# MMAThijssen/catfish

Hardware: AMD Instinct MI355X
Metric: signal samples/s classified (higher is better)
Workload: dtype f32

## Files before the change

catfish_amd/build.py:

```python
from __future__ import annotations

import json
import os
import re
import shutil
import subprocess
import sys

_HERE = os.path.dirname(os.path.abspath(__file__))
SRC = os.path.join(_HERE, "csrc", "catfish_hip.hip")
OUT = os.path.join(_HERE, "csrc", "libcatfish_hip.so")
HEADER = os.path.join(os.path.dirname(_HERE), "include", "catfish_hip.h")


def hipcc_path():
    for cand in (os.environ.get("HIPCC"), shutil.which("hipcc"), "/opt/rocm/bin/hipcc"):
        if cand and os.path.exists(cand):
            return cand
    raise RuntimeError("hipcc not found (set HIPCC or install ROCm)")


def needs_build():
    if not os.path.exists(OUT):
        return True
    csrc = os.path.dirname(SRC)
    deps = [HEADER] + [os.path.join(csrc, f) for f in os.listdir(csrc) if f.endswith((".hip", ".hpp", ".h"))]
    newest = max(os.path.getmtime(p) for p in deps)
    return os.path.getmtime(OUT) < newest


RESOURCES = os.path.join(_HERE, "csrc", "kernel_resources.json")
_REMARK = re.compile(r"remark:\s+(Function Name|TotalSGPRs|VGPRs|AGPRs|ScratchSize \[bytes/lane\]|Occupancy \[waves/SIMD\]|SGPRs Spill|"
                     r"VGPRs Spill|LDS Size \[bytes/block\]):\s*(\S+)")
_KEYS = {"TotalSGPRs": "sgprs", "VGPRs": "vgprs", "AGPRs": "agprs", "ScratchSize [bytes/lane]": "scratch_bytes_per_lane",
         "Occupancy [waves/SIMD]": "waves_per_simd", "SGPRs Spill": "sgpr_spills", "VGPRs Spill": "vgpr_spills",
         "LDS Size [bytes/block]": "lds_bytes"}


def parse_resource_remarks(text):
    out, cur = {}, None
    for m in _REMARK.finditer(text):
        key, val = m.group(1), m.group(2)
        if key == "Function Name":
            cur = out.setdefault(val, {})
        elif cur is not None:
            try:
                cur[_KEYS[key]] = int(val)
            except ValueError:
                pass
    return out


def demangle(names):
    tool = next((t for t in ("/opt/rocm/lib/llvm/bin/llvm-cxxfilt", shutil.which("c++filt")) if t and os.path.exists(t)), None)
    names = list(names)
    if tool is None or not names:
        return dict(zip(names, names))
    res = subprocess.run([tool], input="\n".join(names) + "\n", stdout=subprocess.PIPE, universal_newlines=True)
    got = res.stdout.splitlines()
    return dict(zip(names, got)) if res.returncode == 0 and len(got) == len(names) else dict(zip(names, names))


def check_resources(resources):
    bad = []
    for name, r in sorted(resources.items()):
        if r.get("scratch_bytes_per_lane", 0) != 0 or r.get("vgpr_spills", 0) != 0:
            bad.append("%s: scratch %s B/lane, %s VGPR spills" % (name, r.get("scratch_bytes_per_lane"), r.get("vgpr_spills")))
        if r.get("vgprs", 0) + r.get("agprs", 0) > 512:
            bad.append("%s: %s VGPRs + %s AGPRs exceed the 512-register file" % (name, r.get("vgprs"), r.get("agprs")))
    return bad


def build_native(force=False, verbose=False):
    if not force and not needs_build():
        return OUT
    cmd = [hipcc_path(), "--offload-arch=gfx950", "-O3", "-std=c++17", "-fPIC", "-shared", "-mllvm", "-amdgpu-mfma-vgpr-form",
           "-Rpass-analysis=kernel-resource-usage", "-o", OUT + ".tmp", SRC]
    if verbose:
        print(" ".join(cmd))
    res = subprocess.run(cmd, stdout=subprocess.PIPE, stderr=subprocess.STDOUT, universal_newlines=True)
    if res.returncode != 0:
        if os.path.exists(OUT + ".tmp"):
            os.unlink(OUT + ".tmp")
        raise RuntimeError("hipcc failed:\n" + "\n".join(l for l in res.stdout.splitlines() if "kernel-resource-usage" not in l))
    resources = parse_resource_remarks(res.stdout)
    names = demangle(resources)
    record = {"flags": cmd[1:-3], "kernels": {names[k]: v for k, v in sorted(resources.items())}}
    bad = check_resources(record["kernels"])
    if bad or not resources:
        os.unlink(OUT + ".tmp")
        raise RuntimeError("hipcc built kernels that spill (or reported no kernel resources at all):\n  " + "\n  ".join(bad))
    with open(RESOURCES, "w") as fh:
        json.dump(record, fh, indent=1, sort_keys=True)
        fh.write("\n")
    os.replace(OUT + ".tmp", OUT)
    return OUT


if __name__ == "__main__":
    print(build_native(force="--force" in sys.argv, verbose=True))
```

catfish_amd/csrc/catfish_hip.hip:

```cpp
#include <hip/hip_runtime.h>
#include <stdint.h>
#include <string.h>
#include <stdio.h>
#include <vector>
#include <string>
#include <cmath>
#include <mutex>
#include <set>
#include <functional>

#include "../../include/catfish_hip.h"

typedef float f32x4 __attribute__((ext_vector_type(4)));
typedef float f32x2 __attribute__((ext_vector_type(2)));

#define CF_T 35
#define CF_H 64
#define CF_C 32
#define CF_TILE 16

#define MFMA16(a, b, c) __builtin_amdgcn_mfma_f32_16x16x4f32((a), (b), (c), 0, 0, 0)

#ifndef CF_ABLATE
#define CF_ABLATE 0
#endif
#ifndef CF_PREFETCH
#define CF_PREFETCH 1
#endif

__device__ __forceinline__ float cf_sigmoid(float x) {
    return __builtin_amdgcn_rcpf(1.0f + __expf(-x));
}
__device__ __forceinline__ float cf_tanh(float x) {
    return fmaf(-2.0f, __builtin_amdgcn_rcpf(1.0f + __expf(2.0f * x)), 1.0f);
}
#define CF_GATE_SCALE (-1.4426950408889634)
#define CF_CAND_SCALE (2.8853900817779268)
__device__ __forceinline__ float cf_sigmoid_pre(float a) {
    return __builtin_amdgcn_rcpf(1.0f + __builtin_amdgcn_exp2f(a));
}
__device__ __forceinline__ float cf_tanh_pre(float a) {
    return fmaf(-2.0f, __builtin_amdgcn_rcpf(1.0f + __builtin_amdgcn_exp2f(a)), 1.0f);
}
__device__ __forceinline__ f32x2 cf_sigmoid_pre2(f32x2 a) {
    f32x2 e = {__builtin_amdgcn_exp2f(a.x), __builtin_amdgcn_exp2f(a.y)};
    e = e + (f32x2){1.0f, 1.0f};
    return (f32x2){__builtin_amdgcn_rcpf(e.x), __builtin_amdgcn_rcpf(e.y)};
}
__device__ __forceinline__ f32x2 cf_tanh_pre2(f32x2 a) {
    return __builtin_elementwise_fma((f32x2){-2.0f, -2.0f}, cf_sigmoid_pre2(a), (f32x2){1.0f, 1.0f});
}
template <typename T>
struct far_lds {
    static constexpr int N64K = 65536 / sizeof(T);
    const T *b0, *b1, *b2;
    __device__ __forceinline__ explicit far_lds(const T* base) {
        int o1 = N64K, o2 = 2 * N64K;
        asm volatile("" : "+v"(o1), "+v"(o2));
        b0 = base; b1 = base + o1; b2 = base + o2;
    }
    __device__ __forceinline__ const T& operator[](int e) const { return e < N64K ? b0[e] : (e < 2 * N64K ? b1[e - N64K] : b2[e - 2 * N64K]); }
};
__device__ __forceinline__ f32x4 cf_sigmoid_pre4(f32x4 a) {
    f32x4 e = {__builtin_amdgcn_exp2f(a.x), __builtin_amdgcn_exp2f(a.y), __builtin_amdgcn_exp2f(a.z), __builtin_amdgcn_exp2f(a.w)};
    e = e + (f32x4){1.0f, 1.0f, 1.0f, 1.0f};
    return (f32x4){__builtin_amdgcn_rcpf(e.x), __builtin_amdgcn_rcpf(e.y), __builtin_amdgcn_rcpf(e.z), __builtin_amdgcn_rcpf(e.w)};
}
__device__ __forceinline__ f32x4 cf_tanh_pre4(f32x4 a) {
    return __builtin_elementwise_fma((f32x4){-2.0f, -2.0f, -2.0f, -2.0f}, cf_sigmoid_pre4(a), (f32x4){1.0f, 1.0f, 1.0f, 1.0f});
}
struct cf_dropout {
    float keep_prob = 1.f;
    uint32_t seed = 0;
    int32_t layer = 0;
    const double* step = nullptr;
};
__device__ __forceinline__ uint32_t cf_fmix32(uint32_t v) {
    v ^= v >> 16; v *= 0x85ebca6bu; v ^= v >> 13; v *= 0xc2b2ae35u; v ^= v >> 16;
    return v;
}
__device__ __forceinline__ uint32_t cf_drop_key(const cf_dropout& d) {
    const uint32_t st = d.step ? (uint32_t)(long long)d.step[0] : 0u;
    return cf_fmix32(d.seed ^ cf_fmix32(0x9E3779B9u * (uint32_t)(d.layer + 1) + st * 0x85ebca6bu));
}
__device__ __forceinline__ f32x4 cf_drop_scale4(uint32_t key, float keep_prob, int64_t idx4) {
    const uint32_t thresh = (uint32_t)fminf(keep_prob * 4294967296.0f, 4294967040.0f);
    const float inv = 1.0f / keep_prob;
    const uint64_t e = (uint64_t)idx4 * 4u;
    const uint32_t base = (uint32_t)e ^ ((uint32_t)(e >> 32) * 0x9E3779B9u);
    f32x4 o;
    o.x = cf_fmix32((base + 0u) ^ key) < thresh ? inv : 0.f;
    o.y = cf_fmix32((base + 1u) ^ key) < thresh ? inv : 0.f;
    o.z = cf_fmix32((base + 2u) ^ key) < thresh ? inv : 0.f;
    o.w = cf_fmix32((base + 3u) ^ key) < thresh ? inv : 0.f;
    return o;
}

__device__ __forceinline__ f32x4 relu4(f32x4 v) {
    f32x4 o;
    o.x = fmaxf(v.x, 0.f); o.y = fmaxf(v.y, 0.f); o.z = fmaxf(v.z, 0.f); o.w = fmaxf(v.w, 0.f);
    return o;
}

__host__ __device__ constexpr int gru_x_floats(int cin) { return (cin / 4) * 3 * 256; }
__host__ __device__ constexpr int gru_hg_floats() { return 16 * 2 * 256; }
__host__ __device__ constexpr int gru_hc_floats() { return 16 * 256; }
__host__ __device__ constexpr int gru_bias_off(int cin) { return gru_x_floats(cin) + gru_hg_floats() + gru_hc_floats(); }
__host__ __device__ constexpr int gru_dense_off(int cin) { return gru_bias_off(cin) + 192; }
__host__ __device__ constexpr int gru_pack_floats(int cin) { return gru_dense_off(cin) + 64; }
#define CF_GRU_MAX_WAVES 8
// ... 135 lines not shown
    if (!CHUNKED) t_chunks = 1;
    const int chunk_len = CHUNKED ? (CF_T + t_chunks - 1) / t_chunks : CF_T;
    for (int task = blockIdx.x * waves_per_block + wave; task < n_tiles * t_chunks; task += gridDim.x * waves_per_block) {
        const int tile = CHUNKED ? task / t_chunks : task;
        const int p0 = CHUNKED ? (task - tile * t_chunks) * chunk_len : 0;
        const int p1 = CHUNKED ? min(p0 + chunk_len, CF_T) : CF_T;
        if (CHUNKED && p0 >= p1) continue;
        {
            const int64_t base = (int64_t)tile * CF_TILE * CF_T;
            const int64_t limit = n_windows * CF_T;
            for (int i = lane; i < CF_TILE * CF_T; i += 64) xs[i] = (base + i < limit) ? x_nat[base + i] : 0.f;
            __builtin_amdgcn_fence(__ATOMIC_RELEASE, "wavefront");
            __builtin_amdgcn_wave_barrier();
            __builtin_amdgcn_fence(__ATOMIC_ACQUIRE, "wavefront");
        }
        f32x4 w_sc[2], b_sc[2], w_f[2], b_f[2];
#pragma unroll
        for (int mo = 0; mo < 2; ++mo) { w_sc[mo] = vec0(2, mo); b_sc[mo] = vec0(3, mo); w_f[mo] = vec0(4, mo); b_f[mo] = vec0(5, mo); }
        f32x4 a_pp[2] = {zero, zero}, a_p[2] = {zero, zero}, a_sp[2] = {zero, zero};
        f32x4 b_pp[2] = {zero, zero}, b_p[2] = {zero, zero}, b_sp[2] = {zero, zero};
        for (int i = p0 > 2 ? p0 - 2 : 0; i <= p1 + 1; ++i) {
            f32x4 a_c[2] = {zero, zero}, a_sc[2] = {zero, zero};
            if (i < CF_T) {
                const float xv = xs[(lane & 15) * CF_T + i];
#pragma unroll
                for (int mo = 0; mo < 2; ++mo) {
                    a_sc[mo] = w_sc[mo] * xv + b_sc[mo];
                    a_c[mo] = relu4(w_f[mo] * xv + b_f[mo]);
                }
            }
            f32x4 y0[2] = {zero, zero};
            const bool have_y0 = i >= 1 && i <= CF_T && i >= p0;
            if (have_y0) {
                f32x4 acc[2] = {vec0(0, 0), vec0(0, 1)};
                unit_mma(w0 + 0 * 1024, lane, a_pp, acc);
                unit_mma(w0 + 1 * 1024, lane, a_p, acc);
                unit_mma(w0 + 2 * 1024, lane, a_c, acc);
                f32x4 o2[2] = {relu4(acc[0]), relu4(acc[1])};
                f32x4 acc3[2] = {vec0(1, 0), vec0(1, 1)};
                unit_mma(w0 + 3 * 1024, lane, o2, acc3);
                y0[0] = relu4(relu4(acc3[0]) + a_sp[0]);
                y0[1] = relu4(relu4(acc3[1]) + a_sp[1]);
                if (CHUNKED && y0_frag && i - 1 >= p0 && i - 1 < p1) {
                    f32x4* d0 = y0_frag + ((int64_t)tile * CF_T + (i - 1)) * 2 * 64 + lane;
                    d0[0] = y0[0];
                    d0[64] = y0[1];
                }
            }
            f32x4 b_c[2] = {zero, zero}, b_sc[2] = {zero, zero};
            if (have_y0) {
                b_sc[0] = vec1(0, 0); b_sc[1] = vec1(0, 1);
                unit_mma(w1 + 0 * 1024, lane, y0, b_sc);
                f32x4 acc[2] = {vec1(1, 0), vec1(1, 1)};
                unit_mma(w1 + 1 * 1024, lane, y0, acc);
                b_c[0] = relu4(acc[0]); b_c[1] = relu4(acc[1]);
            }
            if (i >= 2 && i - 2 >= p0 && i - 2 < p1) {
                f32x4 acc[2] = {vec1(2, 0), vec1(2, 1)};
                unit_mma(w1 + 2 * 1024, lane, b_pp, acc);
                unit_mma(w1 + 3 * 1024, lane, b_p, acc);
                unit_mma(w1 + 4 * 1024, lane, b_c, acc);
                f32x4 o2[2] = {relu4(acc[0]), relu4(acc[1])};
                f32x4 acc3[2] = {vec1(3, 0), vec1(3, 1)};
                unit_mma(w1 + 5 * 1024, lane, o2, acc3);
                f32x4* dst = y_frag + ((int64_t)tile * CF_T + (i - 2)) * 2 * 64 + lane;
                dst[0] = relu4(relu4(acc3[0]) + b_sp[0]);
                dst[64] = relu4(relu4(acc3[1]) + b_sp[1]);
            }
#pragma unroll
            for (int mo = 0; mo < 2; ++mo) {
                a_pp[mo] = a_p[mo]; a_p[mo] = a_c[mo]; a_sp[mo] = a_sc[mo];
                if (i >= 1) { b_pp[mo] = b_p[mo]; b_p[mo] = b_c[mo]; b_sp[mo] = b_sc[mo]; }
            }
        }
        __builtin_amdgcn_wave_barrier();
    }
}

template <int CIN>
__device__ __forceinline__ void gru_stage_weights(float* lds, const float* __restrict__ wpack, int dir) {
    constexpr int PACK = gru_pack_floats(CIN);
    const f32x4* src = reinterpret_cast<const f32x4*>(wpack + (size_t)dir * PACK);
    f32x4* dst = reinterpret_cast<f32x4*>(lds);
    for (int i = threadIdx.x; i < PACK / 4; i += blockDim.x) dst[i] = src[i];
}

#ifndef CF_SCHED_DS_FIRST
#define CF_SCHED_DS_FIRST 1
#endif
#if CF_SCHED_DS_FIRST
#define CF_KSTEP_SCHED(nds, nmfma)                               \
    __builtin_amdgcn_sched_group_barrier(0x100, nds, 0);         \
    __builtin_amdgcn_sched_group_barrier(0x008, nmfma, 0);       \
    __builtin_amdgcn_sched_barrier(0)
#else
#define CF_KSTEP_SCHED(nds, nmfma) __builtin_amdgcn_sched_barrier(0)
#endif
template <int CIN, bool LAST, bool STASH = false>
__device__ __forceinline__ void gru_tile(const float* lds, int lane, int dir, int tile, const f32x4* __restrict__ X,
                                         f32x4* __restrict__ Y, float* __restrict__ P, int n_tiles,
                                         f32x4* __restrict__ S = nullptr, f32x4* __restrict__ YD = nullptr, cf_dropout drop = cf_dropout(),
                                         int s_begin = 0, int s_end = CF_T, f32x4* HO = nullptr) {
    const uint32_t drop_key = (STASH && YD) ? cf_drop_key(drop) : 0u;
    constexpr int KGX = CIN / 16;
    constexpr int KSX = CIN / 4;
    constexpr int XN4 = gru_x_floats(CIN) / 4;
    constexpr int HG4 = gru_hg_floats() / 4;
    constexpr int BIAS = gru_bias_off(CIN);
    constexpr int DENSE = gru_dense_off(CIN);
    const int q = lane >> 4;
    const f32x4* WX = reinterpret_cast<const f32x4*>(lds) + lane;
    const far_lds<f32x4> WL(WX);
    const f32x4* B4 = reinterpret_cast<const f32x4*>(lds + BIAS) + q;
    const f32x4* D4 = reinterpret_cast<const f32x4*>(lds + DENSE) + q;
    {
        f32x4 h[4] = {{0, 0, 0, 0}, {0, 0, 0, 0}, {0, 0, 0, 0}, {0, 0, 0, 0}};
        if (s_begin > 0) {
#pragma unroll
            for (int m = 0; m < 4; ++m) h[m] = HO[m * 64 + lane];
        }
        f32x4 xc[KGX];
        {
            const int t0 = dir ? (CF_T - 1 - s_begin) : s_begin;
            const f32x4* src = X + ((int64_t)tile * CF_T + t0) * KGX * 64 + lane;
#pragma unroll
            for (int g = 0; g < KGX; ++g) xc[g] = src[g * 64];
        }
        for (int s = s_begin; s < s_end; ++s) {
            const int t = dir ? (CF_T - 1 - s) : s;
            f32x4 acc[12];
#pragma unroll
            for (int mo = 0; mo < 12; ++mo) acc[mo] = B4[mo * 4];
            constexpr int PF = CF_PREFETCH;
            auto loadA = [&](int p, f32x4 (&d)[3]) {
                if (p < KSX) { d[0] = WL[(p * 3 + 0) * 64]; d[1] = WL[(p * 3 + 1) * 64]; d[2] = WL[(p * 3 + 2) * 64]; }
                else if (p < KSX + 16) { d[0] = WL[XN4 + ((p - KSX) * 2 + 0) * 64]; d[1] = WL[XN4 + ((p - KSX) * 2 + 1) * 64]; }
                else if (p < KSX + 32) { d[0] = WL[XN4 + HG4 + (p - KSX - 16) * 64]; }
            };
            f32x4 ac[3], an[3], a2[3];
            loadA(0, ac);
            if (PF == 2) loadA(1, an);
#pragma unroll
            for (int ks = 0; ks < KSX; ++ks) {
                if (PF == 2) loadA(ks + 2, a2); else loadA(ks + 1, an);
                const float b = xc[ks >> 2][ks & 3];
#pragma unroll
                for (int g = 0; g < 3; ++g) {
                    acc[4 * g + 0] = MFMA16(ac[g].x, b, acc[4 * g + 0]);
                    acc[4 * g + 1] = MFMA16(ac[g].y, b, acc[4 * g + 1]);
                    acc[4 * g + 2] = MFMA16(ac[g].z, b, acc[4 * g + 2]);
                    acc[4 * g + 3] = MFMA16(ac[g].w, b, acc[4 * g + 3]);
                }
                CF_KSTEP_SCHED(3, 12);
#pragma unroll
                for (int g = 0; g < 3; ++g) { ac[g] = an[g]; if (PF == 2) an[g] = a2[g]; }
            }
            {
                int tn = dir ? (t - 1) : (t + 1);
                tn = tn < 0 ? 0 : (tn > CF_T - 1 ? CF_T - 1 : tn);
                const f32x4* src = X + ((int64_t)tile * CF_T + tn) * KGX * 64 + lane;
#pragma unroll
                for (int g = 0; g < KGX; ++g) if (!(CF_ABLATE & 2)) xc[g] = src[g * 64];
            }
#pragma unroll
            for (int ks = 0; ks < 16; ++ks) {
                if (PF == 2) loadA(KSX + ks + 2, a2); else loadA(KSX + ks + 1, an);
                const float b = h[ks >> 2][ks & 3];
#pragma unroll
                for (int g = 0; g < 2; ++g) {
                    acc[4 * g + 0] = MFMA16(ac[g].x, b, acc[4 * g + 0]);
                    acc[4 * g + 1] = MFMA16(ac[g].y, b, acc[4 * g + 1]);
                    acc[4 * g + 2] = MFMA16(ac[g].z, b, acc[4 * g + 2]);
                    acc[4 * g + 3] = MFMA16(ac[g].w, b, acc[4 * g + 3]);
                }
                CF_KSTEP_SCHED(2, 8);
                ac[0] = an[0]; ac[1] = an[1];
                if (PF == 2) { an[0] = a2[0]; an[1] = a2[1]; }
            }
            f32x4 rh[4];
#pragma unroll
            for (int m = 0; m < 4; ++m) {
                if (CF_ABLATE & 1) { rh[m] = acc[m] * 0.001f; continue; }
                const f32x4 rv = cf_sigmoid_pre4(acc[m]);
                rh[m] = rv * h[m];
                if constexpr (STASH) acc[m] = rv;
            }
#pragma unroll
            for (int ks = 0; ks < 16; ++ks) {
                if (PF == 2) loadA(KSX + 16 + ks + 2, a2); else loadA(KSX + 16 + ks + 1, an);
                const float b = rh[ks >> 2][ks & 3];
                acc[8] = MFMA16(ac[0].x, b, acc[8]);
                acc[9] = MFMA16(ac[0].y, b, acc[9]);
                acc[10] = MFMA16(ac[0].z, b, acc[10]);
                acc[11] = MFMA16(ac[0].w, b, acc[11]);
                CF_KSTEP_SCHED(1, 4);
                ac[0] = an[0];
                if (PF == 2) an[0] = a2[0];
            }
#pragma unroll
            for (int m = 0; m < 4; ++m) {
                if (CF_ABLATE & 1) { h[m] = acc[4 + m] * 0.001f + acc[8 + m] * 0.001f; continue; }
                const f32x4 u = cf_sigmoid_pre4(acc[4 + m]);
                const f32x4 c = cf_tanh_pre4(acc[8 + m]);
                h[m] = __builtin_elementwise_fma(u, h[m] - c, c);
                if constexpr (STASH) { acc[4 + m] = u; acc[8 + m] = c; }
            }
            if constexpr (STASH) {
                f32x4* sdst = S + (((int64_t)tile * CF_T + t) * 2 + dir) * 12 * 64 + lane;
#pragma unroll
                for (int j = 0; j < 12; ++j) sdst[j * 64] = acc[j];
            }
            if constexpr (!LAST) {
                f32x4* dst = Y + (((int64_t)tile * CF_T + t) * 8 + dir * 4) * 64 + lane;
#pragma unroll
                for (int m = 0; m < 4; ++m) if (!(CF_ABLATE & 2) || s == CF_T - 1) dst[m * 64] = h[m];
                if constexpr (STASH) {
                    if (YD) {
                        const int64_t i0 = (((int64_t)tile * CF_T + t) * 8 + dir * 4) * 64 + lane;
#pragma unroll
                        for (int m = 0; m < 4; ++m) YD[i0 + m * 64] = h[m] * cf_drop_scale4(drop_key, drop.keep_prob, i0 + m * 64);
                    }
                }
            } else {
                float pm[4];
#pragma unroll
                for (int m = 0; m < 4; ++m) {
                    const f32x4 wd = D4[m * 4];
                    pm[m] = wd.x * h[m].x;
                    pm[m] = fmaf(wd.y, h[m].y, pm[m]); pm[m] = fmaf(wd.z, h[m].z, pm[m]); pm[m] = fmaf(wd.w, h[m].w, pm[m]);
                }
                float p = ((pm[0] + pm[1]) + pm[2]) + pm[3];
                p += __shfl_xor(p, 16);
                p += __shfl_xor(p, 32);
                if (lane < 16) P[(((int64_t)dir * n_tiles + tile) * CF_T + t) * 16 + lane] = p;
            }
            __builtin_amdgcn_sched_barrier(0);
        }
        if (s_end < CF_T) {
#pragma unroll
            for (int m = 0; m < 4; ++m) HO[m * 64 + lane] = h[m];
        }
    }
}

__device__ __forceinline__ void cf_handoff_publish(unsigned* flag) {
    asm volatile("s_waitcnt vmcnt(0)" ::: "memory");
    __builtin_amdgcn_fence(__ATOMIC_RELEASE, "workgroup");
    asm volatile("s_waitcnt vmcnt(0)" ::: "memory");
    __hip_atomic_store(flag, 1u, __ATOMIC_RELAXED, __HIP_MEMORY_SCOPE_WORKGROUP);
}
__device__ __forceinline__ void cf_handoff_wait(unsigned* flag, int lane, unsigned* err) {
    if (lane == 0) {
        bool ok = false;
        for (int it = 0; it < 1000000 && !ok; ++it) {
            ok = __hip_atomic_load(flag, __ATOMIC_RELAXED, __HIP_MEMORY_SCOPE_WORKGROUP) != 0u;
            if (!ok) __builtin_amdgcn_s_sleep(16);
        }
        if (!ok && err) __hip_atomic_store(err, 1u, __ATOMIC_RELAXED, __HIP_MEMORY_SCOPE_SYSTEM);
    }
    __builtin_amdgcn_fence(__ATOMIC_ACQUIRE, "workgroup");
    asm volatile("s_waitcnt vmcnt(0)" ::: "memory");
}

template <int CIN, bool LAST>
__global__ __launch_bounds__(512, 2) void gru_layer_kernel(const float* __restrict__ wpack,
                                                           const f32x4* __restrict__ X,
                                                           f32x4* __restrict__ Y,
                                                           float* __restrict__ P,
                                                           int n_tiles,
                                                           int balance,
                                                           f32x4* hand,
                                                           unsigned* err) {
    extern __shared__ __attribute__((aligned(16))) float lds[];
    const int dir = blockIdx.y;
    gru_stage_weights<CIN>(lds, wpack, dir);
    unsigned* flags = reinterpret_cast<unsigned*>(lds + gru_pack_floats(CIN));
    if (threadIdx.x < CF_GRU_MAX_WAVES) flags[threadIdx.x] = 0u;
    __syncthreads();
    const int lane = threadIdx.x & 63;
    const int wave = __builtin_amdgcn_readfirstlane(threadIdx.x >> 6);
    const int nwaves = blockDim.x >> 6;
    const int t0 = (int)((int64_t)blockIdx.x * n_tiles / gridDim.x);
    const int t1 = (int)((int64_t)(blockIdx.x + 1) * n_tiles / gridDim.x);
    cf_gru_share sh;
    int n_pieces;
    if (balance) {
        sh = cf_gru_balanced_share(t1 - t0, nwaves, wave, CF_T);
        n_pieces = (sh.head_end > 0) + sh.whole_count + (sh.tail_begin < CF_T);
    } else {
        sh.head_tile = sh.head_end = 0; sh.whole_first = sh.whole_count = 0; sh.tail_tile = 0; sh.tail_begin = CF_T;
        n_pieces = t1 - t0 > wave ? (t1 - t0 - wave + nwaves - 1) / nwaves : 0;
    }
    f32x4* slots = hand + ((size_t)(dir * gridDim.x + blockIdx.x) * CF_GRU_MAX_WAVES) * 4 * 64;
    const int has_head = balance && sh.head_end > 0;
    for (int i = 0; i < n_pieces; ++i) {
        int tile, s_begin = 0, s_end = CF_T;
        f32x4* ho = nullptr;
        if (!balance) {
            tile = t0 + wave + i * nwaves;
        } else if (i < has_head) {
            tile = t0 + sh.head_tile; s_end = sh.head_end; ho = slots + wave * 4 * 64;
        } else if (i < has_head + sh.whole_count) {
            tile = t0 + sh.whole_first + (i - has_head);
        } else {
            tile = t0 + sh.tail_tile; s_begin = sh.tail_begin; ho = slots + (wave - 1) * 4 * 64;
            cf_handoff_wait(flags + (wave - 1), lane, err);
        }
        gru_tile<CIN, LAST>(lds, lane, dir, tile, X, Y, P, n_tiles, nullptr, nullptr, cf_dropout(), s_begin, s_end, ho);
        if (s_end < CF_T) cf_handoff_publish(flags + wave);
    }
}

struct cf_fused_args {
    const float* w[3];
    const f32x4* x0;
    f32x4* y[2];
    float* p;
    unsigned* flags;
    int lds_floats;
    unsigned* err;
    int n_tiles;
    int groups;
    int n_layers;
    int cin0;
// ... 792 lines not shown
    *idx = m->ev_pending.size() - 1;
    return CF_OK;
}
static int prof_end(cf_model* m, hipStream_t s, size_t idx) {
    if (!m->prof) return CF_OK;
    HIP_TRY(hipEventRecord(m->ev_pending[idx].b, s));
    return CF_OK;
}

static int pick_waves(int n_tile_tasks, int n_cu) {
    int w = (n_tile_tasks + n_cu - 1) / n_cu;
    return w <= 1 ? 1 : (w <= 2 ? 2 : (w <= 4 ? 4 : 8));
}

static bool use_coop(const cf_model* m, int n_tiles) {
    static const int coop_env = cf_knob("CATFISH_COOP") ? atoi(cf_knob("CATFISH_COOP")) : -1;
    const bool coop = coop_env >= 0 ? coop_env != 0 : n_tiles <= m->n_cu;
    return coop && !(CF_ABLATE & 4) && n_tiles <= m->n_cu;
}

template <int CIN>
static void launch_xproj(cf_model* m, const float* wpack, const float* X, int n_tiles, hipStream_t s) {
    const int lds_env = cf_knob("CATFISH_XPROJ_LDS") ? atoi(cf_knob("CATFISH_XPROJ_LDS")) : 1;
    if (lds_env) {
        int chunks = cf_xproj_plan(n_tiles, m->n_cu, CIN);
        if (cf_knob("CATFISH_XPROJ_CHUNKS")) {
            const int c = std::max(1, std::min(CF_T, atoi(cf_knob("CATFISH_XPROJ_CHUNKS"))));
            const int tl = (CF_T + c - 1) / c;
            chunks = (CF_T + tl - 1) / tl;
        }
        hipLaunchKernelGGL((gru_xproj_lds_kernel<CIN>), dim3(n_tiles * chunks, 2), dim3(256), gru_x_floats(CIN) * 4, s, wpack,
                           reinterpret_cast<const f32x4*>(X), reinterpret_cast<f32x4*>(m->d_xp), n_tiles, chunks);
    } else {
        hipLaunchKernelGGL((gru_xproj_kernel<CIN>), dim3(n_tiles * cf_xproj_chunks(n_tiles), 2), dim3(256), 0, s, wpack,
                           reinterpret_cast<const f32x4*>(X), reinterpret_cast<f32x4*>(m->d_xp), n_tiles, cf_xproj_chunks(n_tiles));
    }
}

template <int CIN, bool LAST>
static int launch_gru(cf_model* m, const float* wpack, const float* X, float* Y, float* P, int n_tiles, hipStream_t s, int slot,
                      float* hand = nullptr) {
    if (use_coop(m, n_tiles)) {
        size_t pi = 0;
        int rc = prof_begin(m, slot, s, &pi);
        if (rc != CF_OK) return rc;
        const int gx = std::min(n_tiles, std::max(1, m->n_cu / 2));
        const f32x4* xp = nullptr;
        if (CIN >= 32 && n_tiles <= m->xp_tiles) {
            xp = reinterpret_cast<const f32x4*>(m->d_xp);
            launch_xproj<CIN>(m, wpack, X, n_tiles, s);
        }
        hipLaunchKernelGGL((gru_layer_coop_kernel<CIN, LAST>), dim3(gx, 2), dim3(256), (gru_pack_floats(CIN) + CF_COOP_XCH_FLOATS) * 4, s,
                           wpack, reinterpret_cast<const f32x4*>(X), reinterpret_cast<f32x4*>(Y), P, n_tiles, xp);
        HIP_TRY(hipGetLastError());
        return prof_end(m, s, pi);
    }
    static const int waves_env = cf_knob("CATFISH_WAVES") ? atoi(cf_knob("CATFISH_WAVES")) : 0;
    const int waves = waves_env > 0 ? std::min(waves_env, 8) : ((CF_ABLATE & 4) ? 4 : pick_waves(2 * n_tiles, m->n_cu));
    const int groups = (n_tiles + waves - 1) / waves;
    int per_dir = m->n_cu / 2 > 0 ? m->n_cu / 2 : 1;
    constexpr int lds_bytes = gru_pack_floats(CIN) * 4;
    if (lds_bytes <= 80 * 1024) per_dir *= 2;
    int gx = groups < per_dir ? groups : per_dir;
    size_t pi = 0;
    int rc = prof_begin(m, slot, s, &pi);
    if (rc != CF_OK) return rc;
    int balance = 0;
    if (hand) {
        const int wg_per_cu = std::max(1, (2 * gx + m->n_cu - 1) / m->n_cu);
        const int gx_one = std::max(1, m->n_cu / 2);
        const int load_rr = cf_gru_grid_load(n_tiles, gx, waves, wg_per_cu, CF_T, 0);
        const int load_bal = cf_gru_grid_load(n_tiles, gx, waves, wg_per_cu, CF_T, 1);
        const int load_one = gx > gx_one ? cf_gru_grid_load(n_tiles, gx_one, waves, 1, CF_T, 1) : -1;
        const char* env = cf_knob("CATFISH_GRU_BALANCE");
        const int forced = env ? atoi(env) : -1;
        int best = load_rr;
        if (forced < 0 ? (load_bal >= 0 && load_bal < best) : (forced >= 1 && load_bal >= 0)) { balance = 1; best = load_bal; }
        if (forced < 0 ? (load_one >= 0 && load_one < best) : (forced == 2 && load_one >= 0)) { balance = 1; gx = gx_one; }
    }
    hipLaunchKernelGGL((gru_layer_kernel<CIN, LAST>), dim3(gx, 2), dim3(waves * 64), lds_bytes + CF_GRU_MAX_WAVES * 4, s, wpack,
                       reinterpret_cast<const f32x4*>(X), reinterpret_cast<f32x4*>(Y), P, n_tiles, balance, reinterpret_cast<f32x4*>(hand),
                       m->d_err);
    HIP_TRY(hipGetLastError());
    return prof_end(m, s, pi);
}

template <int CIN, bool LAST, int NP>
static int launch_gru_bf16(cf_model* m, const char* wpack, const float* X, float* Y, float* P, int n_tiles32, hipStream_t s, int slot) {
    static const int waves_env = cf_knob("CATFISH_BF16_WAVES") ? atoi(cf_knob("CATFISH_BF16_WAVES")) : 0;
    static const int wgs_env = cf_knob("CATFISH_BF16_WGS") ? atoi(cf_knob("CATFISH_BF16_WGS")) : 0;
    const int waves = waves_env > 0 ? std::min(waves_env, 8) : pick_waves(2 * n_tiles32, m->n_cu);
    const int groups = (n_tiles32 + waves - 1) / waves;
    int per_dir = m->n_cu / 2 > 0 ? m->n_cu / 2 : 1;
    constexpr int lds_bytes = gb_pack_bytes(CIN, NP);
    if (lds_bytes <= 80 * 1024) per_dir *= 2;
    if (wgs_env > 0) per_dir = wgs_env;
    const int gx = groups < per_dir ? groups : per_dir;
    size_t pi = 0;
    int rc = prof_begin(m, slot, s, &pi);
    if (rc != CF_OK) return rc;
    const int pipe_env = cf_knob("CATFISH_BF16_PIPE") ? atoi(cf_knob("CATFISH_BF16_PIPE")) : 1;
    if constexpr (NP == 1) {
        if (pipe_env) {
            hipLaunchKernelGGL((gru_bf16_pipe_kernel<CIN, LAST>), dim3(gx, 2), dim3(waves * 64), lds_bytes, s, wpack,
                               reinterpret_cast<const bf16x8*>(X), reinterpret_cast<bf16x8*>(Y), P, n_tiles32);
            HIP_TRY(hipGetLastError());
            return prof_end(m, s, pi);
        }
    }
    if constexpr (NP == 2) {
        if (pipe_env) {
            const int w4 = std::min(waves, 4);
            const int g4 = (n_tiles32 + w4 - 1) / w4;
            const int per4 = wgs_env > 0 ? wgs_env : std::max(1, m->n_cu / 2);
            hipLaunchKernelGGL((gru_bf16x3_pipe_kernel<CIN, LAST>), dim3(std::min(g4, per4), 2), dim3(w4 * 64), lds_bytes, s, wpack,
                               reinterpret_cast<const bf16x8*>(X), reinterpret_cast<bf16x8*>(Y), P, n_tiles32);
            HIP_TRY(hipGetLastError());
            return prof_end(m, s, pi);
        }
    }
    hipLaunchKernelGGL((gru_layer_bf16_kernel<CIN, LAST, NP>), dim3(gx, 2), dim3(waves * 64), lds_bytes, s, wpack,
                       reinterpret_cast<const bf16x8*>(X), reinterpret_cast<bf16x8*>(Y), P, n_tiles32);
    HIP_TRY(hipGetLastError());
    return prof_end(m, s, pi);
}

template <int NP>
static int launch_gru_bf16_layer(cf_model* m, int l, bool last, const float* cur, float* y, float* p, int n_tiles32, hipStream_t s) {
    const char* wp = m->d_gru_b[l];
    if (l == 0)
        return last ? launch_gru_bf16<32, true, NP>(m, wp, cur, y, p, n_tiles32, s, SLOT_GRU_LAST)
                    : launch_gru_bf16<32, false, NP>(m, wp, cur, y, p, n_tiles32, s, SLOT_GRU0);
    return last ? launch_gru_bf16<128, true, NP>(m, wp, cur, y, p, n_tiles32, s, SLOT_GRU_LAST)
                : launch_gru_bf16<128, false, NP>(m, wp, cur, y, p, n_tiles32, s, SLOT_GRU);
}

#include "generic_host.hpp"
#include "params_dev.hpp"

static int cf_fuse_min_groups(int n_cu) { return 6 * std::max(1, n_cu / 2); }

static int run_pass(cf_model* m, cf_model::Slot& sl, const float* x, int64_t n_windows, float* probs, float* logits, hipStream_t s) {
    const int n_tiles = (int)((n_windows + CF_TILE - 1) / CF_TILE);
    const int n_tiles32 = (int)((n_windows + 2 * CF_TILE - 1) / (2 * CF_TILE));
    int rc;
    size_t pi = 0;
    const bool res_split = m->np == 0 && n_tiles <= m->n_cu;
    const int res_chunks = res_split ? 4 : 1;
    const int res_waves = res_split ? 4 : (pick_waves(n_tiles, m->n_cu * 2) > 4 ? 4 : pick_waves(n_tiles, m->n_cu * 2));
    const int res_grid = res_split ? n_tiles : std::min((n_tiles + res_waves - 1) / res_waves, m->n_cu * 4);
    const int res_fuse_env = cf_knob("CATFISH_RES_FUSE") ? atoi(cf_knob("CATFISH_RES_FUSE")) : 1;
    const bool res_fused = m->np == 0 && m->hp.n_layers_res >= 2 && res_fuse_env != 0;
    const bool res_fused_bf16 = m->np > 0 && m->hp.n_layers_res >= 2 && res_fuse_env != 0;
    sl.last_res_fused = (res_fused && !res_split) || res_fused_bf16;
    if (res_fused_bf16) {
        if ((rc = prof_begin(m, SLOT_RES_STACK2, s, &pi)) != CF_OK) return rc;
        const int np = m->np > 1 ? 2 : 1;
        const int tpw = (np == 1 && cf_knob("CATFISH_RES_TPW") && atoi(cf_knob("CATFISH_RES_TPW")) == 2) ? 2 : 1;
        const int groups = (n_tiles32 + tpw - 1) / tpw;
        const int slots = (np == 1 && tpw == 1 ? 4 * CF_RES_BF16_WAVES : 8) * m->n_cu;
        int chunks = std::max(1, std::min(CF_T, slots / std::max(1, groups)));
        if (cf_knob("CATFISH_RES_CHUNKS")) chunks = std::max(1, std::min(CF_T, atoi(cf_knob("CATFISH_RES_CHUNKS"))));
        const int len = (CF_T + chunks - 1) / chunks;
        chunks = (CF_T + len - 1) / len;
        const int lds_bytes = rb_pack_bytes(true, np) + rb_pack_bytes(false, np) + 4 * tpw * 32 * CF_T * 4;
        const int per_cu = std::max(1, std::min(np == 1 && tpw == 1 ? CF_RES_BF16_WAVES : 2, (160 * 1024) / lds_bytes));
// ... 855 lines not shown
```

Baseline: 341.3 million.

## Defer GRU output stores, specialize zero-state first step, batch weight staging loads

Each GRU timestep's output store (hidden state or projection) is now issued during the next step, after the input-side MFMAs, so the global write overlaps compute instead of sitting at the end of the step. The first timestep gets a compile-time specialization that skips the recurrent MFMAs, since the hidden state starts at zero. Weight staging into LDS now issues a batch of global loads before the LDS writes so more loads are in flight. A disabled timing-stamp instrumentation path and a build helper for define variants are also added.

```diff
diff --git a/catfish_amd/build.py b/catfish_amd/build.py
--- a/catfish_amd/build.py
+++ b/catfish_amd/build.py
@@ -71,30 +71,35 @@
     return bad
 
 
-def build_native(force=False, verbose=False):
-    if not force and not needs_build():
+def build_native(force=False, verbose=False, out=None, defines=()):
+    variant = out is not None or bool(defines)
+    if variant and out is None:
+        raise ValueError("a build with -D defines needs its own output path")
+    if not variant and not force and not needs_build():
         return OUT
+    dest = os.path.abspath(out) if variant else OUT
     cmd = [hipcc_path(), "--offload-arch=gfx950", "-O3", "-std=c++17", "-fPIC", "-shared", "-mllvm", "-amdgpu-mfma-vgpr-form",
-           "-Rpass-analysis=kernel-resource-usage", "-o", OUT + ".tmp", SRC]
+           "-Rpass-analysis=kernel-resource-usage"] + ["-D%s" % d for d in defines] + ["-o", dest + ".tmp", SRC]
     if verbose:
         print(" ".join(cmd))
     res = subprocess.run(cmd, stdout=subprocess.PIPE, stderr=subprocess.STDOUT, universal_newlines=True)
     if res.returncode != 0:
-        if os.path.exists(OUT + ".tmp"):
-            os.unlink(OUT + ".tmp")
+        if os.path.exists(dest + ".tmp"):
+            os.unlink(dest + ".tmp")
         raise RuntimeError("hipcc failed:\n" + "\n".join(l for l in res.stdout.splitlines() if "kernel-resource-usage" not in l))
     resources = parse_resource_remarks(res.stdout)
     names = demangle(resources)
     record = {"flags": cmd[1:-3], "kernels": {names[k]: v for k, v in sorted(resources.items())}}
     bad = check_resources(record["kernels"])
     if bad or not resources:
-        os.unlink(OUT + ".tmp")
+        os.unlink(dest + ".tmp")
         raise RuntimeError("hipcc built kernels that spill (or reported no kernel resources at all):\n  " + "\n  ".join(bad))
-    with open(RESOURCES, "w") as fh:
-        json.dump(record, fh, indent=1, sort_keys=True)
-        fh.write("\n")
-    os.replace(OUT + ".tmp", OUT)
-    return OUT
+    if not variant:
+        with open(RESOURCES, "w") as fh:
+            json.dump(record, fh, indent=1, sort_keys=True)
+            fh.write("\n")
+    os.replace(dest + ".tmp", dest)
+    return dest
 
 
 if __name__ == "__main__":
diff --git a/catfish_amd/csrc/catfish_hip.hip b/catfish_amd/csrc/catfish_hip.hip
--- a/catfish_amd/csrc/catfish_hip.hip
+++ b/catfish_amd/csrc/catfish_hip.hip
@@ -26,6 +26,15 @@
 #endif
 #ifndef CF_PREFETCH
 #define CF_PREFETCH 1
+#endif
+#ifndef CF_GRU_DEFER_STORE
+#define CF_GRU_DEFER_STORE 1
+#endif
+#ifndef CF_GRU_STEP0
+#define CF_GRU_STEP0 1
+#endif
+#ifndef CF_GRU_STAGE_INFLIGHT
+#define CF_GRU_STAGE_INFLIGHT 1
 #endif
 
 __device__ __forceinline__ float cf_sigmoid(float x) {
@@ -327,11 +336,45 @@
     constexpr int PACK = gru_pack_floats(CIN);
     const f32x4* src = reinterpret_cast<const f32x4*>(wpack + (size_t)dir * PACK);
     f32x4* dst = reinterpret_cast<f32x4*>(lds);
+#if CF_GRU_STAGE_INFLIGHT
+    constexpr int N4 = PACK / 4;
+    constexpr int BATCH = (N4 + 511) / 512;
+    for (int base = threadIdx.x; base < N4; base += BATCH * blockDim.x) {
+        f32x4 v[BATCH];
+#pragma unroll
+        for (int j = 0; j < BATCH; ++j) { const int i = base + j * blockDim.x; v[j] = src[i < N4 ? i : N4 - 1]; }
+#pragma unroll
+        for (int j = 0; j < BATCH; ++j) { const int i = base + j * blockDim.x; if (i < N4) dst[i] = v[j]; }
+    }
+#else
     for (int i = threadIdx.x; i < PACK / 4; i += blockDim.x) dst[i] = src[i];
+#endif
 }
 
 #ifndef CF_SCHED_DS_FIRST
 #define CF_SCHED_DS_FIRST 1
+#endif
+#ifndef CF_GRU_STAMP
+#define CF_GRU_STAMP 0
+#endif
+#if CF_GRU_STAMP
+__device__ unsigned long long cf_gru_stamp_acc[3];
+#define CF_GRU_STAMP_TOP()                                                              \
+    {                                                                                   \
+        __builtin_amdgcn_sched_barrier(0);                                              \
+        const long long ta_ = (long long)__builtin_amdgcn_s_memtime();                  \
+        asm volatile("s_waitcnt lgkmcnt(0)\n\ts_waitcnt vmcnt(0)" ::: "memory");        \
+        const long long tb_ = (long long)__builtin_amdgcn_s_memtime();                  \
+        asm volatile("s_waitcnt lgkmcnt(0)" ::: "memory");                              \
+        const long long tc_ = (long long)__builtin_amdgcn_s_memtime();                  \
+        asm volatile("s_waitcnt lgkmcnt(0)" ::: "memory");                              \
+        const long long td_ = (long long)__builtin_amdgcn_s_memtime();                  \
+        asm volatile("s_waitcnt lgkmcnt(0)" ::: "memory");                              \
+        st_wait_ += tb_ - ta_; st_ref_ += td_ - tc_; ++st_n_;                           \
+        __builtin_amdgcn_sched_barrier(0);                                              \
+    }
+#else
+#define CF_GRU_STAMP_TOP()
 #endif
 #if CF_SCHED_DS_FIRST
 #define CF_KSTEP_SCHED(nds, nmfma)                               \
@@ -371,14 +414,31 @@
 #pragma unroll
             for (int g = 0; g < KGX; ++g) xc[g] = src[g * 64];
         }
-        for (int s = s_begin; s < s_end; ++s) {
+        constexpr bool DEFER = CF_GRU_DEFER_STORE && !STASH;
+#if CF_GRU_STAMP
+        long long st_wait_ = 0, st_ref_ = 0, st_n_ = 0;
+#endif
+        float p_out = 0.f;
+        auto store_out = [&](int s, int t) {
+            if constexpr (!LAST) {
+                f32x4* dst = Y + (((int64_t)tile * CF_T + t) * 8 + dir * 4) * 64 + lane;
+#pragma unroll
+                for (int m = 0; m < 4; ++m) if (!(CF_ABLATE & 2) || s == CF_T - 1) dst[m * 64] = h[m];
+            } else {
+                if (lane < 16) P[(((int64_t)dir * n_tiles + tile) * CF_T + t) * 16 + lane] = p_out;
+            }
+        };
+        auto step = [&](auto zero_h, const int s) {
+            constexpr bool ZERO_H = decltype(zero_h)::value;
             const int t = dir ? (CF_T - 1 - s) : s;
+            CF_GRU_STAMP_TOP();
             f32x4 acc[12];
 #pragma unroll
             for (int mo = 0; mo < 12; ++mo) acc[mo] = B4[mo * 4];
             constexpr int PF = CF_PREFETCH;
             auto loadA = [&](int p, f32x4 (&d)[3]) {
                 if (p < KSX) { d[0] = WL[(p * 3 + 0) * 64]; d[1] = WL[(p * 3 + 1) * 64]; d[2] = WL[(p * 3 + 2) * 64]; }
+                else if (ZERO_H) { }
                 else if (p < KSX + 16) { d[0] = WL[XN4 + ((p - KSX) * 2 + 0) * 64]; d[1] = WL[XN4 + ((p - KSX) * 2 + 1) * 64]; }
                 else if (p < KSX + 32) { d[0] = WL[XN4 + HG4 + (p - KSX - 16) * 64]; }
             };
@@ -400,6 +460,9 @@
 #pragma unroll
                 for (int g = 0; g < 3; ++g) { ac[g] = an[g]; if (PF == 2) an[g] = a2[g]; }
             }
+            if constexpr (DEFER && !ZERO_H) {
+                if (s > s_begin) store_out(s - 1, dir ? (t + 1) : (t - 1));
+            }
             {
                 int tn = dir ? (t - 1) : (t + 1);
                 tn = tn < 0 ? 0 : (tn > CF_T - 1 ? CF_T - 1 : tn);
@@ -407,47 +470,55 @@
 #pragma unroll
                 for (int g = 0; g < KGX; ++g) if (!(CF_ABLATE & 2)) xc[g] = src[g * 64];
             }
-#pragma unroll
-            for (int ks = 0; ks < 16; ++ks) {
-                if (PF == 2) loadA(KSX + ks + 2, a2); else loadA(KSX + ks + 1, an);
-                const float b = h[ks >> 2][ks & 3];
-#pragma unroll
-                for (int g = 0; g < 2; ++g) {
-                    acc[4 * g + 0] = MFMA16(ac[g].x, b, acc[4 * g + 0]);
-                    acc[4 * g + 1] = MFMA16(ac[g].y, b, acc[4 * g + 1]);
-                    acc[4 * g + 2] = MFMA16(ac[g].z, b, acc[4 * g + 2]);
-                    acc[4 * g + 3] = MFMA16(ac[g].w, b, acc[4 * g + 3]);
+            if constexpr (!ZERO_H) {
+#pragma unroll
+                for (int ks = 0; ks < 16; ++ks) {
+                    if (PF == 2) loadA(KSX + ks + 2, a2); else loadA(KSX + ks + 1, an);
+                    const float b = h[ks >> 2][ks & 3];
+#pragma unroll
+                    for (int g = 0; g < 2; ++g) {
+                        acc[4 * g + 0] = MFMA16(ac[g].x, b, acc[4 * g + 0]);
+                        acc[4 * g + 1] = MFMA16(ac[g].y, b, acc[4 * g + 1]);
+                        acc[4 * g + 2] = MFMA16(ac[g].z, b, acc[4 * g + 2]);
+                        acc[4 * g + 3] = MFMA16(ac[g].w, b, acc[4 * g + 3]);
+                    }
+                    CF_KSTEP_SCHED(2, 8);
+                    ac[0] = an[0]; ac[1] = an[1];
+                    if (PF == 2) { an[0] = a2[0]; an[1] = a2[1]; }
                 }
-                CF_KSTEP_SCHED(2, 8);
-                ac[0] = an[0]; ac[1] = an[1];
-                if (PF == 2) { an[0] = a2[0]; an[1] = a2[1]; }
             }
-            f32x4 rh[4];
-#pragma unroll
-            for (int m = 0; m < 4; ++m) {
-                if (CF_ABLATE & 1) { rh[m] = acc[m] * 0.001f; continue; }
-                const f32x4 rv = cf_sigmoid_pre4(acc[m]);
-                rh[m] = rv * h[m];
-                if constexpr (STASH) acc[m] = rv;
-            }
-#pragma unroll
-            for (int ks = 0; ks < 16; ++ks) {
-                if (PF == 2) loadA(KSX + 16 + ks + 2, a2); else loadA(KSX + 16 + ks + 1, an);
-                const float b = rh[ks >> 2][ks & 3];
-                acc[8] = MFMA16(ac[0].x, b, acc[8]);
-                acc[9] = MFMA16(ac[0].y, b, acc[9]);
-                acc[10] = MFMA16(ac[0].z, b, acc[10]);
-                acc[11] = MFMA16(ac[0].w, b, acc[11]);
-                CF_KSTEP_SCHED(1, 4);
-                ac[0] = an[0];
-                if (PF == 2) an[0] = a2[0];
+            if constexpr (!ZERO_H) {
+                f32x4 rh[4];
+#pragma unroll
+                for (int m = 0; m < 4; ++m) {
+                    if (CF_ABLATE & 1) { rh[m] = acc[m] * 0.001f; continue; }
+                    const f32x4 rv = cf_sigmoid_pre4(acc[m]);
+                    rh[m] = rv * h[m];
+                    if constexpr (STASH) acc[m] = rv;
+                }
+#pragma unroll
+                for (int ks = 0; ks < 16; ++ks) {
+                    if (PF == 2) loadA(KSX + 16 + ks + 2, a2); else loadA(KSX + 16 + ks + 1, an);
+                    const float b = rh[ks >> 2][ks & 3];
+                    acc[8] = MFMA16(ac[0].x, b, acc[8]);
+                    acc[9] = MFMA16(ac[0].y, b, acc[9]);
+                    acc[10] = MFMA16(ac[0].z, b, acc[10]);
+                    acc[11] = MFMA16(ac[0].w, b, acc[11]);
+                    CF_KSTEP_SCHED(1, 4);
+                    ac[0] = an[0];
+                    if (PF == 2) an[0] = a2[0];
+                }
+            } else if constexpr (STASH) {
+#pragma unroll
+                for (int m = 0; m < 4; ++m) acc[m] = cf_sigmoid_pre4(acc[m]);
             }
 #pragma unroll
             for (int m = 0; m < 4; ++m) {
                 if (CF_ABLATE & 1) { h[m] = acc[4 + m] * 0.001f + acc[8 + m] * 0.001f; continue; }
                 const f32x4 u = cf_sigmoid_pre4(acc[4 + m]);
                 const f32x4 c = cf_tanh_pre4(acc[8 + m]);
-                h[m] = __builtin_elementwise_fma(u, h[m] - c, c);
+                const f32x4 hp = ZERO_H ? (f32x4){0, 0, 0, 0} : h[m];
+                h[m] = __builtin_elementwise_fma(u, hp - c, c);
                 if constexpr (STASH) { acc[4 + m] = u; acc[8 + m] = c; }
             }
             if constexpr (STASH) {
@@ -456,9 +527,7 @@
                 for (int j = 0; j < 12; ++j) sdst[j * 64] = acc[j];
             }
             if constexpr (!LAST) {
-                f32x4* dst = Y + (((int64_t)tile * CF_T + t) * 8 + dir * 4) * 64 + lane;
-#pragma unroll
-                for (int m = 0; m < 4; ++m) if (!(CF_ABLATE & 2) || s == CF_T - 1) dst[m * 64] = h[m];
+                if constexpr (!DEFER) store_out(s, t);
                 if constexpr (STASH) {
                     if (YD) {
                         const int64_t i0 = (((int64_t)tile * CF_T + t) * 8 + dir * 4) * 64 + lane;
@@ -477,14 +546,30 @@
                 float p = ((pm[0] + pm[1]) + pm[2]) + pm[3];
                 p += __shfl_xor(p, 16);
                 p += __shfl_xor(p, 32);
-                if (lane < 16) P[(((int64_t)dir * n_tiles + tile) * CF_T + t) * 16 + lane] = p;
+                p_out = p;
+                if constexpr (!DEFER) store_out(s, t);
             }
             __builtin_amdgcn_sched_barrier(0);
+        };
+        int s = s_begin;
+#if CF_GRU_STEP0
+        if (s_begin == 0 && s_end > 0) { step(std::true_type(), 0); s = 1; }
+#endif
+        for (; s < s_end; ++s) step(std::false_type(), s);
+        if constexpr (DEFER) {
+            if (s_end > s_begin) store_out(s_end - 1, dir ? (CF_T - s_end) : (s_end - 1));
         }
         if (s_end < CF_T) {
 #pragma unroll
             for (int m = 0; m < 4; ++m) HO[m * 64 + lane] = h[m];
         }
+#if CF_GRU_STAMP
+        if (lane == 0) {
+            atomicAdd(&cf_gru_stamp_acc[0], (unsigned long long)st_wait_);
+            atomicAdd(&cf_gru_stamp_acc[1], (unsigned long long)st_ref_);
+            atomicAdd(&cf_gru_stamp_acc[2], (unsigned long long)st_n_);
+        }
+#endif
     }
 }
 
@@ -1443,6 +1528,18 @@
                        reinterpret_cast<const f32x4*>(X), reinterpret_cast<f32x4*>(Y), P, n_tiles, balance, reinterpret_cast<f32x4*>(hand),
                        m->d_err);
     HIP_TRY(hipGetLastError());
+#if CF_GRU_STAMP
+    {
+        static int launches = 0;
+        if (++launches % 90 == 0) {
+            unsigned long long acc[3];
+            HIP_TRY(hipStreamSynchronize(s));
+            HIP_TRY(hipMemcpyFromSymbol(acc, HIP_SYMBOL(cf_gru_stamp_acc), sizeof(acc)));
+            fprintf(stderr, "gru stamp after %d launches: %llu wave-steps, top-of-step wait %.1f cycles, empty stamp pair %.1f cycles\n", launches,
+                    acc[2], (double)acc[0] / (double)acc[2], (double)acc[1] / (double)acc[2]);
+        }
+    }
+#endif
     return prof_end(m, s, pi);
 }
 
```

Result: faster. 348.5 million, median of 6 (+2.1%).
